# yanyan-li/Structure-SLAM-PointLine

Measured on AMD Instinct MI355X. Metric: front-end frames/sec (ORB+LSD extract+match) 640x480 @1000kp/200ln, higher is better.
Workload: dtype u8; 1 GPU; BASELINE configs[2]: 640x480 ORB(1000kp,8 levels)+LSD/LBD(<=200 lines) extract + Hamming match vs previous frame, inputs resident in HBM; batch_per_gpu=12288, global_batch=12288, unique_frames=64, streams=point branch and line branch on two HIP streams, parallelism=single GPU

## Files before the change

structure-slam-pointline_amd/csrc/lbd.h:

```cpp
#pragma once

template <class KeyPtr>
__device__ __forceinline__ void keyline_sort(KeyPtr keys, int P2, int tid) {
    for (int k = 2; k <= P2; k <<= 1)
        for (int j = k >> 1; j > 0; j >>= 1) {
            for (int i = tid; i < P2; i += 256) {
                int ixj = i ^ j;
                if (ixj > i) {
                    unsigned long long a = keys[i], c = keys[ixj];
                    bool up = (i & k) == 0;
                    if ((a > c) == up) { keys[i] = c; keys[ixj] = a; }
                }
            }
            __syncthreads();
        }
}

constexpr int KL_LDS = 1024;
__global__ __launch_bounds__(256) void k_keylines(uint8_t* __restrict__ ws, LsdPlan P, int maxLines,
                                                  sslam_keyline* __restrict__ klOut, double* __restrict__ fnOut,
                                                  int* __restrict__ counts, int cap) {
    __shared__ unsigned long long keysL[KL_LDS];
    const int b = blockIdx.x, tid = threadIdx.x;
    uint8_t* base = ws + (size_t)b * P.frameBytes;
// ... 33 lines not shown
        const float W = (float)P.w, H = (float)P.h;
        if (e0 < 0) e0 = 0; if (e0 >= W) e0 = W - 1.0f;
        if (e2 < 0) e2 = 0; if (e2 >= W) e2 = W - 1.0f;
        if (e1 < 0) e1 = 0; if (e1 >= H) e1 = H - 1.0f;
        if (e3 < 0) e3 = 0; if (e3 >= H) e3 = H - 1.0f;
        sslam_keyline k;
        k.startPointX = e0; k.startPointY = e1; k.endPointX = e2; k.endPointY = e3;
        k.sPointInOctaveX = e0; k.sPointInOctaveY = e1; k.ePointInOctaveX = e2; k.ePointInOctaveY = e3;
        const double ddx = (double)__fsub_rn(e0, e2), ddy = (double)__fsub_rn(e1, e3);
        k.lineLength = (float)sqrt(ddx * ddx + ddy * ddy);
        const int ax = cv_roundf(e0), ay = cv_roundf(e1), bx = cv_roundf(e2), by = cv_roundf(e3);
        k.numOfPixels = max(abs(bx - ax), abs(by - ay)) + 1;
        k.angle = (float)atan2((double)__fsub_rn(e3, e1), (double)__fsub_rn(e2, e0));
        k.class_id = i; k.octave = 0;
        k.size = __fmul_rn(__fsub_rn(e2, e0), __fsub_rn(e3, e1));
        k.response = __fdiv_rn(k.lineLength, (float)max(P.w, P.h));
        k.pt_x = __fdiv_rn(__fadd_rn(e2, e0), 2.f); k.pt_y = __fdiv_rn(__fadd_rn(e3, e1), 2.f);
        klw[i] = k;
        const unsigned long long key = ((unsigned long long)(~__float_as_uint(k.response)) << 32) | (unsigned)i;
        if (inLds) keysL[i] = key; else keysG[i] = key;
    }
    __syncthreads();
    int nOut = n;
    const bool doSort = n > maxLines;
    if (doSort) {
        int P2 = 1; while (P2 < n) P2 <<= 1;
        if (inLds) {
            for (int i = n + tid; i < P2; i += 256) keysL[i] = ~0ull;
            __syncthreads();
            keyline_sort(keysL, P2, tid);
        } else {
            for (int i = n + tid; i < P2; i += 256) keysG[i] = ~0ull;
            __syncthreads();
            keyline_sort(keysG, P2, tid);
        }
        nOut = maxLines;
    }
    nOut = min(nOut, cap);
    for (int i = tid; i < nOut; i += 256) {
        const int src = doSort ? (int)(unsigned)(inLds ? keysL[i] : keysG[i]) : i;
        sslam_keyline k = klw[src];
        if (doSort) k.class_id = i;
        klOut[(size_t)b * cap + i] = k;
        ((float2*)(base + P.offLbdDir))[i] = make_float2((float)cos((double)k.angle), (float)sin((double)k.angle));
        const double sx = k.startPointX, sy = k.startPointY, ex = k.endPointX, ey = k.endPointY;
        const double l0 = __dsub_rn(sy, ey), l1 = __dsub_rn(ex, sx), l2 = __dsub_rn(__dmul_rn(sx, ey), __dmul_rn(sy, ex));
        const double nrm = sqrt(__dadd_rn(__dmul_rn(l0, l0), __dmul_rn(l1, l1)));
        double* f = fnOut + ((size_t)b * cap + i) * 3;
        f[0] = l0 / nrm; f[1] = l1 / nrm; f[2] = l2 / nrm;
    }
    if (tid == 0) { counts[b] = nOut; misc->nKl = nOut; }
}

__global__ __launch_bounds__(256) void k_blur_sobel(const uint8_t* __restrict__ src, size_t spitch, size_t sframe, int w, int h,
                                                    unsigned* __restrict__ dxyo, size_t dframeBytes,
                                                    const int* __restrict__ tapsArr) {
    constexpr int R = 3;
    const int ngroups = (w + 3) >> 2;
    const int t = blockIdx.x * 256 + threadIdx.x;
    const int strip = t / ngroups, x4 = (t - strip * ngroups) * 4, y0 = strip * STRIP;
    if (y0 >= h) return;
    const int b = blockIdx.y;
    const uint8_t* s = src + (size_t)b * sframe;
    unsigned taps[5];
#pragma unroll
    for (int k = 0; k < 5; ++k) taps[k] = (unsigned)tapsArr[k];
    const unsigned T0 = taps[0] | (taps[1] << 8) | (taps[2] << 16) | (taps[3] << 24), T1 = taps[4];
    const bool fast = x4 >= 4 && x4 + 8 <= w && ((spitch | (size_t)(uintptr_t)s) & 3) == 0;
    const bool vec = ((w & 3) == 0) && ((dframeBytes & 15) == 0);
    unsigned hb[5][6];
    int bl[3][6];
    constexpr int NR = STRIP + 2 * R;
    const bool uni = row12_uniform(s, spitch, w);
    const int x4u = uni ? x4 : 0;
    Row12 ring[ROW_AHEAD_SOBEL];
#pragma unroll
    for (int k = 0; k < ROW_AHEAD_SOBEL; ++k) ring[k] = row12_issue(s, spitch, reflect_row(y0 - R + k, h, R), x4u, w);
#pragma unroll
    for (int r = 0; r < NR; ++r) {
        if (r >= 2 * R && y0 + r - 2 * R >= h) break;
        Row12 cur = ring[r % ROW_AHEAD_SOBEL];
        if (r + ROW_AHEAD_SOBEL < NR) ring[r % ROW_AHEAD_SOBEL] = row12_issue(s, spitch, reflect_row(y0 - R + r + ROW_AHEAD_SOBEL, h, R), x4u, w);
        row12_fix(cur, x4u, w);
        if (!uni) load_row12(s, spitch, reflect_row(y0 - R + r, h, R), x4, w, fast, cur.d0, cur.d1, cur.d2);
        const unsigned d0 = cur.d0, d1 = cur.d1, d2 = cur.d2;
#pragma unroll
        for (int c = 0; c < 6; ++c) hb[r % 5][c] = hdot(d0, d1, d2, c + 1, T0, T1);
        if (r >= 4) {
            const int q = r - 4;
#pragma unroll
            for (int c = 0; c < 6; ++c) {
                unsigned acc = 0;
#pragma unroll
                for (int k = 0; k < 5; ++k) acc = __umul24(hb[(q + k) % 5][c], taps[k]) + acc;
                bl[q % 3][c] = (int)min((acc + 32768u) >> 16, 255u);
            }
            if (q >= 2) {
                const int y = y0 + q - 2;
                const int* A = bl[(q - 2) % 3];
                const int* M = bl[(q - 1) % 3];
                const int* C = bl[q % 3];
                short gx[4], gy[4];
#pragma unroll
                for (int j = 0; j < 4; ++j) {
                    gx[j] = (short)((A[j + 2] - A[j]) + 2 * (M[j + 2] - M[j]) + (C[j + 2] - C[j]));
                    gy[j] = (short)((C[j] - A[j]) + 2 * (C[j + 1] - A[j + 1]) + (C[j + 2] - A[j + 2]));
                }
                unsigned* op = (unsigned*)((uint8_t*)dxyo + (size_t)b * dframeBytes) + (size_t)y * w + x4;
                unsigned pk[4];
#pragma unroll
                for (int j = 0; j < 4; ++j) pk[j] = ((unsigned)(unsigned short)gx[j]) | ((unsigned)(unsigned short)gy[j] << 16);
                if (x4 + 3 < w && vec) *(uint4*)op = make_uint4(pk[0], pk[1], pk[2], pk[3]);
                else {
#pragma unroll
                    for (int j = 0; j < 4; ++j) if (x4 + j < w) op[j] = pk[j];
                }
            }
        }
    }
}

__constant__ float kGaussL[21];
__constant__ float kGaussL2[21];
__constant__ float kGaussG[63];
__constant__ signed char kComb[64];

typedef float f32x2 __attribute__((ext_vector_type(2)));
__device__ __forceinline__ int cvt_rpi(float x) { int r; asm("v_cvt_rpi_i32_f32 %0, %1" : "=v"(r) : "v"(x)); return r; }
__device__ __forceinline__ f32x2 pk_mul_lo(f32x2 a, f32x2 b) { f32x2 r; asm("v_pk_mul_f32 %0, %1, %2 op_sel:[0,0] op_sel_hi:[1,0]" : "=v"(r) : "v"(a), "v"(b)); return r; }
__device__ __forceinline__ f32x2 pk_mul_hi_swapped(f32x2 a, f32x2 b) { f32x2 r; asm("v_pk_mul_f32 %0, %1, %2 op_sel:[1,1] op_sel_hi:[0,1]" : "=v"(r) : "v"(a), "v"(b)); return r; }
__device__ __forceinline__ f32x2 pk_add_sub(f32x2 a, f32x2 b) { f32x2 r; asm("v_pk_add_f32 %0, %1, %2 neg_hi:[0,1]" : "=v"(r) : "v"(a), "v"(b)); return r; }
__device__ __forceinline__ f32x2 pk_sub(f32x2 a, f32x2 b) { f32x2 r; asm("v_pk_add_f32 %0, %1, %2 neg_lo:[0,1] neg_hi:[0,1]" : "=v"(r) : "v"(a), "v"(b)); return r; }
__device__ __forceinline__ float max0(float x) { float r; asm("v_max_f32 %0, 0, %1" : "=v"(r) : "v"(x)); return r; }
__device__ __forceinline__ int med3_0(int x, int hi) { int r; asm("v_med3_i32 %0, %1, 0, %2" : "=v"(r) : "v"(x), "s"(hi)); return r; }
__device__ __forceinline__ f32x2 pk_mul(f32x2 a, f32x2 b) { f32x2 r; asm("v_pk_mul_f32 %0, %1, %2" : "=v"(r) : "v"(a), "v"(b)); return r; }
__device__ __forceinline__ f32x2 pk_add(f32x2 a, f32x2 b) { f32x2 r; asm("v_pk_add_f32 %0, %1, %2" : "=v"(r) : "v"(a), "v"(b)); return r; }

#ifdef SSLAM_TESTING
__global__ __launch_bounds__(256) void k_selftest_lbd_round(unsigned long long* __restrict__ bad) {
    unsigned long long nb0 = 0, nb1 = 0;
    const unsigned base = (blockIdx.x * 256u + threadIdx.x) << 8;
    for (unsigned i = 0; i < 256u; ++i) {
        const float x = __uint_as_float(base + i);
        if (!(fabsf(x) < 24608.f)) continue;
        const int t = (int)__fadd_rn(x, x);
        const int o = (int)(short)((t + 1) >> 1), n = cvt_rpi(x);
        const int Ws[3] = {0, 639, 16383};
#pragma unroll
        for (int k = 0; k < 3; ++k) nb0 += (min(max(o, 0), Ws[k]) != min(max(n, 0), Ws[k])) ? 1 : 0;
        if (x >= 0.f) nb1 += (n != (int)roundf(x)) ? 1 : 0;
    }
    if (nb0) atomicAdd(bad, nb0);
    if (nb1) atomicAdd(bad + 1, nb1);
}
#endif
constexpr int LBD_TB = 8;
template <bool RPI>
__global__ __launch_bounds__(64) void k_lbd(const uint8_t* __restrict__ ws, LsdPlan P, const sslam_keyline* __restrict__ kls,
                                            const int* __restrict__ counts, uint8_t* __restrict__ descOut, int cap) {
    constexpr int TB = LBD_TB, TN = TB, TP = TB + 1;
    __shared__ unsigned tbuf[64 * TP];
    float (*rows)[64] = (float (*)[64])&tbuf[0];
    static_assert(8 * 64 <= 64 * TP, "rows[][] lies over the walk's block array");
    __shared__ float band[8][NUM_BANDS];
    __shared__ float des[72];
    const int li = blockIdx.x, b = blockIdx.y, lane = threadIdx.x;
    if (li >= counts[b]) return;
    const uint8_t* base = ws + (size_t)b * P.frameBytes;
    const unsigned* dxyImg = (const unsigned*)(base + P.offDxy);
    const sslam_keyline kl = kls[(size_t)b * cap + li];
    const int lengthOfLSP = (short)kl.numOfPixels;
// ... 177 lines not shown
```

structure-slam-pointline_amd/csrc/lines.hip:

```cpp
#include "common.h"
#include <cmath>
#include <cstdlib>
#include <cfloat>
#include <algorithm>

namespace sslam { int launch_nfa_stream(sslam_ctx* ctx, hipStream_t st, uint8_t* ws, const void* plan, size_t planBytes, const double* lgam, uint8_t* clArea, size_t clFrameBytes,
                                        size_t stageOff, int nframes, int waves, long long spinTicks, bool besideCore); }
namespace sslam { int launch_nfa_stage(sslam_ctx* ctx, hipStream_t st, uint8_t* ws, const void* plan, size_t planBytes, const double* lgam, int nframes); }

using namespace sslam;

namespace {

#include "lsd_plan.h"
#include "lsd_front.h"
#include "lsd_regions.h"
#include "lsd_cluster.h"
#include "lsd_nfa.h"
#include "lbd.h"

__global__ void k_zero_misc(uint8_t* ws, LsdPlan P) {
    Misc* m = (Misc*)(ws + (size_t)blockIdx.x * P.frameBytes + P.offMisc);
    if (threadIdx.x == 0) {
        m->maxS = 0; m->nDefined = 0; m->nSeg = 0; m->nCand = 0; m->nKl = 0; m->overflow = 0; m->claim = 0;
// ... 119 lines not shown
    };
    P.nfaVariant = L->nfaVariant; P.lbdBitOrder = L->lbdBitOrder; P.lsdResize = L->lsdResize;
    P.tabX = 0; if (P.lsdResize) coeffs_linear(w, P.sw); else coeffs(SCALE, w, P.sw);
    P.tabY = (int)tabs.size(); if (P.lsdResize) coeffs_linear(h, P.sh); else coeffs(SCALE, h, P.sh);
    int rc;
    if ((rc = L->dTabs.ensure(tabs.size() * sizeof(int)))) return rc;
    SSLAM_HIP(hipMemcpy(L->dTabs.p, tabs.data(), tabs.size() * sizeof(int), hipMemcpyHostToDevice));
    int taps[16] = {0};
    for (int i = 0; i < 7; ++i) taps[i] = t7[i];
    for (int i = 0; i < 5; ++i) taps[8 + i] = t5[i];
    if ((rc = L->dTaps.ensure(sizeof(taps)))) return rc;
    SSLAM_HIP(hipMemcpy(L->dTaps.p, taps, sizeof(taps), hipMemcpyHostToDevice));
    size_t off = 0;
    auto take = [&](size_t bytes) { size_t o = off; off = align_up(off + bytes, 256); return o; };
    const size_t bpitch = ((size_t)w + 63) & ~(size_t)63;
    P.offBlur = take(bpitch * h);
    P.tW = P.sw; P.cW = P.sw;
    P.offT = take(sizeof(float) * (size_t)P.npx);
    P.offS = take(sizeof(int) * (size_t)P.npx);
    P.offCs = take(sizeof(float2) * (size_t)P.npx);
    P.offOrder = take(sizeof(unsigned) * (size_t)P.npx);
    P.offTileHist = take(sizeof(int) * (size_t)P.nTiles * N_BINS);
    P.offReg = take(sizeof(unsigned) * std::max((size_t)P.npx, (size_t)P.sh * P.nXB * 256));
    P.offComp = P.offReg;
    P.offSegCnt = take(sizeof(int) * (size_t)P.sh * P.nXB);
    P.offSorted = take(sizeof(unsigned) * (size_t)P.sh * P.nXB * 256);
    P.offSeg = take(sizeof(float4) * MAX_SEG);
    P.offCand = take(sizeof(double) * 12 * MAX_SEG);
    P.offFlag = take(sizeof(int) * MAX_SEG);
    P.offNfa = take(sizeof(NfaState) * MAX_SEG);
    P.offMisc = take(sizeof(Misc));
    P.offDxy = take(sizeof(unsigned) * (size_t)w * h);
    P.offKl = take(sizeof(sslam_keyline) * MAX_SEG);
    P.offLbdDir = take(sizeof(float2) * MAX_SEG);
    P.frameBytes = align_up(off, 4096);
    if (!L->dGtab.p) {
        if ((rc = L->dGtab.ensure(sizeof(float4) * ((size_t)GT * GT + 1)))) return rc;
        int* dSmin = (int*)(L->dGtab.as<float4>() + (size_t)GT * GT);
        const int big = 0x7FFFFFFF;
        SSLAM_HIP(hipMemcpy(dSmin, &big, sizeof(int), hipMemcpyHostToDevice));
        hipLaunchKernelGGL(k_grad_table, dim3((GT * GT + 255) / 256), dim3(256), 0, L->ctx->stream, L->dGtab.as<float4>(), P.rho);
        hipLaunchKernelGGL(k_grad_smin, dim3((2 * 510 * 510 + 256) / 256), dim3(256), 0, L->ctx->stream, dSmin, P.rho);
        SSLAM_HIP(hipStreamSynchronize(L->ctx->stream));
        SSLAM_HIP(hipMemcpy(&L->sMin, dSmin, sizeof(int), hipMemcpyDeviceToHost));
    }
    P.sMin = L->sMin;
    {
        const int nl = P.npx + 4;
        if ((rc = L->dLgam.ensure(sizeof(double) * (2 * (size_t)nl + 48)))) return rc;
        if ((rc = upload_nfa_tables(L->dLgam.as<double>(), nl, L->ctx->stream))) return rc;
    }
    {
        bool ok = (w % 4) == 0 && (P.sw % 4) == 0 && (P.sh % 4) == 0 && w == 5 * (P.sw / 4) && h == 5 * (P.sh / 4) && w >= 20 && h >= 10 && t7[0] == 0 && t7[6] == 0;
        for (int x = 0; ok && x < P.sw; ++x) ok = tabs[(size_t)P.tabX + 2 * x] == 5 * (x >> 2) + (x & 3);
        for (int y = 0; ok && y < P.sh; ++y) ok = tabs[(size_t)P.tabY + 2 * y] == 5 * (y >> 2) + (y & 3);
        L->fusedGeometry = ok;
    }
    L->planW = w; L->planH = h; L->wsFrames = 0;
    return SSLAM_OK;
}

extern "C" int sslam_lines_create(sslam_ctx* ctx, int max_lines, sslam_lines** out) {
    if (!ctx || !out || max_lines <= 0 || max_lines > MAX_SEG) { set_error("sslam_lines_create: invalid arguments"); return SSLAM_ERR_INVALID; }
    sslam_lines* L = new sslam_lines();
    L->ctx = ctx; L->maxLines = max_lines;
    *out = L;
    return SSLAM_OK;
}

extern "C" int sslam_lines_set_blur_variant(sslam_lines* L, int variant) {
    if (!L || (variant != 0 && variant != 1)) { set_error("sslam_lines_set_blur_variant: invalid arguments"); return SSLAM_ERR_INVALID; }
    std::lock_guard<std::recursive_mutex> lk(L->ctx->mu);
    if (L->blurVariant != variant) { L->blurVariant = variant; L->planW = L->planH = 0; }
    return SSLAM_OK;
}

static int lines_set_variant(sslam_lines* L, int which, int variant, const char* name) {
    if (!L || (variant != 0 && variant != 1)) { set_error("%s: invalid arguments", name); return SSLAM_ERR_INVALID; }
    std::lock_guard<std::recursive_mutex> lk(L->ctx->mu);
    int& field = which == 0 ? L->nfaVariant : which == 1 ? L->lbdBitOrder : which == 2 ? L->lsdResize : L->seedOrder;
    if (field != variant) { field = variant; L->planW = L->planH = 0; }
    return SSLAM_OK;
}
extern "C" int sslam_lines_set_nfa_variant(sslam_lines* L, int variant) { return lines_set_variant(L, 0, variant, "sslam_lines_set_nfa_variant"); }
extern "C" int sslam_lines_set_lbd_bit_order(sslam_lines* L, int variant) { return lines_set_variant(L, 1, variant, "sslam_lines_set_lbd_bit_order"); }
extern "C" int sslam_lines_set_resize_variant(sslam_lines* L, int variant) { return lines_set_variant(L, 2, variant, "sslam_lines_set_resize_variant"); }
extern "C" int sslam_lines_set_seed_order(sslam_lines* L, int variant) { return lines_set_variant(L, 3, variant, "sslam_lines_set_seed_order"); }

static int lines_host_seed_order(sslam_lines* L, uint8_t* ws, int nframes, hipStream_t st) {
    const LsdPlan& P = L->plan;
    struct NormPoint { int x, y, norm; };
    std::vector<int> S((size_t)P.npx);
    std::vector<NormPoint> pts;
    std::vector<unsigned> order;
    SSLAM_HIP(hipStreamSynchronize(st));
    for (int b = 0; b < nframes; ++b) {
        uint8_t* base = ws + (size_t)b * P.frameBytes;
        Misc m;
        SSLAM_HIP(hipMemcpy(&m, base + P.offMisc, sizeof(m), hipMemcpyDeviceToHost));
        SSLAM_HIP(hipMemcpy(S.data(), base + P.offS, sizeof(int) * (size_t)P.npx, hipMemcpyDeviceToHost));
        const double maxGrad = m.maxS > 0 ? std::sqrt((double)m.maxS / 4.0) : -1.0;
        const double binCoef = maxGrad > 0 ? (double)(N_BINS - 1) / maxGrad : 0.0;
        pts.clear(); pts.reserve((size_t)(P.sw - 1) * (P.sh - 1));
        for (int y = 0; y < P.sh - 1; ++y)
            for (int x = 0; x < P.sw - 1; ++x) pts.push_back({x, y, (int)(std::sqrt((double)S[(size_t)y * P.sw + x] / 4.0) * binCoef)});
        std::sort(pts.begin(), pts.end(), [](const NormPoint& a, const NormPoint& c) { return a.norm > c.norm; });
        order.clear();
// ... 42 lines not shown
enum class CoreForm {
    ClusterStream,
    Cluster,
    Lone,
    Guest,
    PerFrame,
    SixWave,
};

constexpr int CL_MAXFRAMES = 64;

static CoreForm lines_core_form(const sslam_lines* L, const LsdPlan& P, int nframes, const LinesKnobs& K, int* grid) {
    if (K.cluster && nframes <= CL_MAXFRAMES && P.sw <= TorusGlobal::XMASK + 1 && P.sh <= TorusGlobal::YMASK + 1)
        return K.nfaStreamWaves ? CoreForm::ClusterStream : CoreForm::Cluster;
    if (K.lone >= 0 ? K.lone != 0 : nframes < 1024) return CoreForm::Lone;
    if (lines_guest_form(L, nframes, K, grid)) return CoreForm::Guest;
    return nframes <= 16 * L->ctx->num_cus ? CoreForm::PerFrame : CoreForm::SixWave;
}

extern "C" int sslam_lines_destroy(sslam_lines* L) {
    if (!L) return SSLAM_OK;
    (void)hipSetDevice(L->ctx->device);
    (void)hipStreamSynchronize(L->ctx->stream);
    if (L->nfaStream) { (void)hipStreamSynchronize(L->nfaStream); (void)hipStreamDestroy(L->nfaStream); (void)hipEventDestroy(L->nfaFork); (void)hipEventDestroy(L->nfaJoin); }
    DevBuf* bufs[] = {&L->dWs, &L->dCl, &L->dTabs, &L->dTaps, &L->dLgam, &L->dGtab, &L->dImg, &L->dKl, &L->dDesc, &L->dFn, &L->dCounts};
    for (DevBuf* b : bufs) b->release();
    L->hOut.release();
    delete L;
    return SSLAM_OK;
}

struct LinesCall {
    sslam_lines* L; const LsdPlan& P; const uint8_t* images; size_t pitch, imageStride; int nframes; hipStream_t st; uint8_t* ws;
};

struct SideJoin {
    sslam_lines* L; hipStream_t st; bool forked = false, joined = false;
    void join() { if (forked && !joined) { (void)hipEventRecord(L->nfaJoin, L->nfaStream); (void)hipStreamWaitEvent(st, L->nfaJoin, 0); joined = true; } }
    ~SideJoin() { join(); }
};

static int lines_side_stream_ready(sslam_lines* L) {
    if (!L->nfaStream) {
        SSLAM_HIP(hipStreamCreateWithFlags(&L->nfaStream, hipStreamNonBlocking));
        SSLAM_HIP(hipEventCreateWithFlags(&L->nfaFork, hipEventDisableTiming));
        SSLAM_HIP(hipEventCreateWithFlags(&L->nfaJoin, hipEventDisableTiming));
    }
    return SSLAM_OK;
}

static void lines_blur_sobel(const LinesCall& c, hipStream_t s) {
    const LsdPlan& P = c.P;
    sslam::ProfScope _ps(c.L->ctx, "k_blur_sobel", s);
    hipLaunchKernelGGL(k_blur_sobel, dim3((((P.w + 3) / 4) * ((P.h + STRIP - 1) / STRIP) + 255) / 256, c.nframes), dim3(256), 0, s, c.images, c.pitch, c.imageStride, P.w, P.h,
                       (unsigned*)(c.ws + P.offDxy), P.frameBytes, c.L->dTaps.as<int>() + 8);
}

static int lines_prologue(const LinesCall& c) {
    sslam_lines* L = c.L; const LsdPlan& P = c.P; hipStream_t st = c.st;
    const int* taps = L->dTaps.as<int>();
    const int* tabX = L->dTabs.as<int>() + P.tabX; const int* tabY = L->dTabs.as<int>() + P.tabY;
    const int mode = (P.lsdResize ? 1 : 0) | (L->seedOrder ? 2 : 0);
    const bool fused = L->fusedGeometry && GRAD_ROWS == 8 && ((uintptr_t)c.images & 3) == 0 && (c.pitch & 3) == 0 && (c.imageStride & 3) == 0 && c.pitch <= 0x7FFFFFFF;
    if (fused) {
        static decltype(&k_lsd_grad_fused<0>) const kGradFused[4] = {k_lsd_grad_fused<0>, k_lsd_grad_fused<1>, k_lsd_grad_fused<2>, k_lsd_grad_fused<3>};
        sslam::ProfScope _ps(L->ctx, "k_lsd_grad", st);
        const dim3 gg(P.nXB, (P.sh + 31) / 32, c.nframes);
        hipLaunchKernelGGL(kGradFused[mode], gg, dim3(64, 4), 0, st, c.images, c.pitch, c.imageStride, c.ws, P, L->dGtab.as<float4>(), tabX, tabY, taps, c.nframes);
    } else {
        static decltype(&k_lsd_grad<0>) const kGrad[4] = {k_lsd_grad<0>, k_lsd_grad<1>, k_lsd_grad<2>, k_lsd_grad<3>};
        const size_t bpitch = ((size_t)P.w + 63) & ~(size_t)63;
        { sslam::ProfScope _ps(L->ctx, "k_blur7", st); hipLaunchKernelGGL(k_blur7, dim3((((P.w + 3) / 4) * ((P.h + STRIP - 1) / STRIP) + 255) / 256, c.nframes), dim3(256), 0, st, c.images, c.pitch, c.imageStride,
                           c.ws + P.offBlur, bpitch, P.frameBytes, P.w, P.h, taps); }
        { sslam::ProfScope _ps(L->ctx, "k_lsd_grad", st);
          const dim3 gg(P.nXB, (P.sh + 4 * GRAD_ROWS - 1) / (4 * GRAD_ROWS), c.nframes);
          hipLaunchKernelGGL(kGrad[mode], gg, dim3(64, 4), 0, st, c.ws, P, L->dGtab.as<float4>(), bpitch, tabX, tabY); }
    }
    if (L->seedOrder) return lines_host_seed_order(L, c.ws, c.nframes, st);
    const bool runs = P.sw <= (1 << SORT_XY_BITS) && P.sh <= (1 << SORT_XY_BITS);
    const dim3 sg(sort_grid(P.nTiles, c.nframes));
    { sslam::ProfScope _ps(L->ctx, "k_lsd_hist", st); hipLaunchKernelGGL(runs ? k_lsd_hist_sort : k_lsd_hist, sg, dim3(64), 0, st, c.ws, P, c.nframes); }
    { sslam::ProfScope _ps(L->ctx, "k_lsd_scan", st); hipLaunchKernelGGL(k_lsd_scan, dim3(c.nframes), dim3(1024), 0, st, c.ws, P); }
    { sslam::ProfScope _ps(L->ctx, "k_lsd_scatter", st); hipLaunchKernelGGL(runs ? k_lsd_scatter_runs : k_lsd_scatter, sg, dim3(64), 0, st, c.ws, P, c.nframes); }
    return SSLAM_OK;
}

static int lines_core_cluster(const LinesCall& c, const LinesKnobs& K, bool streamNfa, SideJoin& side, size_t* nfaStageOff) {
    sslam_lines* L = c.L; const LsdPlan& P = c.P; const int nframes = c.nframes; hipStream_t st = c.st;
    int rc;
    const bool bigFrame = P.sw > TorusFrame::XMASK + 1 || P.sh > TorusFrame::YMASK + 1;
    const int window = K.clWindow, clShift = K.clSmap;
    int nWG = K.clWgs;
    const int clSpecWords = clShift < 0 ? 0 : (((P.sw + (1 << clShift) - 1) >> clShift) * ((P.sh + (1 << clShift) - 1) >> clShift) + 31) / 32;
    const size_t maxSubs = ((size_t)P.npx + CL_SUB - 1) / CL_SUB;
    const size_t zeroBytes = 512 + ((maxSubs * sizeof(ClSub) + 511) & ~(size_t)511) + 4 * (size_t)((clSpecWords + 127) & ~127) + (bigFrame ? 4 * (size_t)TorusGlobal::WORDS : 0);
    if (nframes > 8) nWG = std::max(2, std::min(nWG, 32 / ((nframes + 7) / 8)));
    const size_t stageOff = zeroBytes + maxSubs * CL_RES * sizeof(ClRec) + 4 * (size_t)CL_ARENA * (size_t)std::max(1, (nWG - 1) * CL_HPW);
    const size_t clFrame = align_up(stageOff + (streamNfa ? sizeof(double) * 12 * (size_t)MAX_SEG : 0), 4096);
    L->clFrame = clFrame; L->clSlots = nframes;
    const size_t clSlots = (size_t)nframes;
    if (L->dCl.cap < clFrame * clSlots) { SSLAM_HIP(hipStreamSynchronize(st)); if ((rc = L->dCl.ensure(clFrame * clSlots))) return rc; }
    for (int f = 0; f < nframes; ++f) SSLAM_HIP(hipMemsetAsync(L->dCl.as<uint8_t>() + (size_t)f * clFrame, 0, zeroBytes, st));
    const size_t clLds = sizeof(unsigned) * std::max((size_t)QCAP + 4 + (bigFrame ? 0 : TorusFrame::WORDS) + CL_SCAN + CL_RING_WORDS, (size_t)CL_HPW * (CL_LIST + ClTorus::WORDS));
    const auto kern = streamNfa ? k_lsd_regions_cl<1> : k_lsd_regions_cl<0>;
    const dim3 grd(8 * nWG * ((nframes + 7) / 8));
    SSLAM_HIP(hipFuncSetAttribute((const void*)kern, hipFuncAttributeMaxDynamicSharedMemorySize, (int)clLds));
    if (!streamNfa) {
        hipLaunchKernelGGL(kern, grd, dim3(64 * CL_WAVES), clLds, st, c.ws, P, L->dCl.as<uint8_t>(), clFrame, nframes, nWG, clSpecWords, clShift, window);
// ... 460 lines not shown
```

structure-slam-pointline_amd/csrc/lsd_front.h:

```cpp
#pragma once

constexpr int STRIP = 32;

__device__ __forceinline__ void load_row12(const uint8_t* __restrict__ s, size_t spitch, int yy, int x4, int w, bool fast, unsigned& d0, unsigned& d1, unsigned& d2) {
    const uint8_t* row = s + (size_t)yy * spitch;
    if (fast) {
        const unsigned* q = (const unsigned*)(row + x4 - 4);
        d0 = q[0]; d1 = q[1]; d2 = q[2];
    } else {
        unsigned px[12];
#pragma unroll
        for (int i = 0; i < 12; ++i) {
            int xx = reflect101(min(x4 - 4 + i, w + 2), w);
            xx = min(max(xx, 0), w - 1);
            px[i] = row[xx];
        }
        d0 = px[0] | (px[1] << 8) | (px[2] << 16) | (px[3] << 24);
        d1 = px[4] | (px[5] << 8) | (px[6] << 16) | (px[7] << 24);
        d2 = px[8] | (px[9] << 8) | (px[10] << 16) | (px[11] << 24);
    }
}
struct Row12 { unsigned d0, d1, d2; };
constexpr int ROW_AHEAD_BLUR7 = 1, ROW_AHEAD_SOBEL = 2;
__device__ __forceinline__ bool row12_uniform(const uint8_t* s, size_t spitch, int w) { return (w & 3) == 0 && w >= 12 && ((spitch | (size_t)(uintptr_t)s) & 3) == 0; }
// ... 183 lines not shown
                float4* c = (float4*)(Cs + i);
                c[0] = make_float4(cs[0].x, cs[0].y, cs[1].x, cs[1].y);
                c[1] = make_float4(cs[2].x, cs[2].y, cs[3].x, cs[3].y);
            }
        } else {
#pragma unroll
            for (int j = 0; j < 4; ++j) if (x4 + j < P.sw) {
                T[i + j] = ang[j];
                if (DENSE) S[i + j] = sv[j];
                if (flags & (1u << j)) { S[i + j] = sv[j]; Cs[i + j] = cs[j]; }
            }
        }
        const int seg = y * P.nXB + blockIdx.x;
        const int cnt = __popc(flags), incl = wave_incl_scan(cnt);
        unsigned* dst = comp + ((size_t)seg << 8);
        int pos = incl - cnt;
#pragma unroll
        for (int j = 0; j < 4; ++j) if (flags & (1u << j)) dst[pos++] = ((unsigned)sv[j] << 8) | (unsigned)(4 * lane + j);
        if (lane == 63) segCnt[seg] = incl;
#pragma unroll
        for (int j = 0; j < 4; ++j) if (!DENSE || (flags & (1u << j))) smax = max(smax, sv[j]);
    };
    int pc[5], pn[5];
    if (fast) {
        unsigned d0[2][3], d1[2][3];
        load_raw(yBeg, d0); load_raw(min(yBeg + 1, P.sh - 1), d1);
        scale_fast(yBeg, d0, pc);
        for (int y = yBeg; y < yEnd; ++y) {
            scale_fast(min(y + 1, P.sh - 1), d1, pn);
            load_raw(min(y + 2, P.sh - 1), d1);
            process(y, pc, pn);
#pragma unroll
            for (int j = 0; j < 5; ++j) pc[j] = pn[j];
        }
    } else {
        scale_slow(yBeg, pc);
        for (int y = yBeg; y < yEnd; ++y) {
            scale_slow(min(y + 1, P.sh - 1), pn);
            process(y, pc, pn);
#pragma unroll
            for (int j = 0; j < 5; ++j) pc[j] = pn[j];
        }
    }
    smax = wave_max(smax);
    if (lane == 0 && smax > 0) atomicMax(&misc->maxS, smax);
}


struct Raw16 { unsigned v[4]; };
template <int MODE>
__global__ __launch_bounds__(256) void k_lsd_grad_fused(const uint8_t* __restrict__ img, size_t ipitch, size_t iframe, const uint8_t* __restrict__ ws, LsdPlan P,
                                                        const float4* __restrict__ gtab, const int* __restrict__ tx, const int* __restrict__ ty, const int* __restrict__ tapsArr, int nframes) {
    constexpr bool LIN = (MODE & 1) != 0, DENSE = (MODE & 2) != 0;
    for (int b = blockIdx.z; b < nframes; b += gridDim.z) {
    const uint8_t* base = ws + (size_t)b * P.frameBytes;
    const uint8_t* src = img + (size_t)b * iframe;
    float* T = (float*)(base + P.offT);
    float2* Cs = (float2*)(base + P.offCs);
    int* S = (int*)(base + P.offS); (void)S;
    Misc* misc = (Misc*)(base + P.offMisc);
    unsigned* comp = (unsigned*)(base + P.offComp);
    int* segCnt = (int*)(base + P.offSegCnt);
    const int lane = threadIdx.x;
    const int strip = __builtin_amdgcn_readfirstlane(blockIdx.y * 4 + threadIdx.y);
    const int yBeg = strip * 8, yEnd = min(P.sh, yBeg + 8);
    if (yBeg >= P.sh) return;
    const int x4 = (blockIdx.x * 64 + lane) * 4;
    const bool inx = x4 < P.sw;
    const int x4c = min(x4, P.sw - 4);
    const int c0 = (x4c >> 2) * 5;
    unsigned cx[5];
#pragma unroll
    for (int j = 0; j < 5; ++j) cx[j] = (unsigned)((const int2*)tx)[min(x4c + j, P.sw - 1)].y;
    const int2* tyv = (const int2*)ty;
    const int a = (c0 - 2) & ~3;
    const unsigned o0 = (unsigned)(c0 - 2) & 3u;
    const bool isLeft = a < 0, isRight = a + 8 >= P.w;
    const int aLoad = isLeft ? 0 : a;
    const unsigned t1 = (unsigned)tapsArr[1], t2 = (unsigned)tapsArr[2], t3 = (unsigned)tapsArr[3], t4 = (unsigned)tapsArr[4], t5 = (unsigned)tapsArr[5];
    const unsigned TA = t1 | (t2 << 8) | (t3 << 16) | (t4 << 24);
    unsigned Hring[5][4];
    const int off2 = min(aLoad + 8, P.w - 4), off3 = min(aLoad + 12, P.w - 4);
    auto raw_row = [&](int n) -> Raw16 {
        const int rr = reflect_row(10 * strip - 2 + n, P.h, 2);
        const uint8_t* row = src + (size_t)rr * ipitch;
        Raw16 r;
        const uint2 lo = *(const uint2*)(row + aLoad);
        r.v[0] = lo.x; r.v[1] = lo.y; r.v[2] = *(const unsigned*)(row + off2); r.v[3] = *(const unsigned*)(row + off3);
        return r;
    };
    auto hrow = [&](const Raw16& r, unsigned (&Hp)[4]) {
        unsigned L0 = r.v[0], L1 = r.v[1], L2 = r.v[2], L3 = r.v[3];
        if (isLeft) {
            L3 = L2; L2 = L1; L1 = L0;
            L0 = __builtin_amdgcn_perm(L2, L1, 0x01020304u);
        }
        if (isRight) L2 = __builtin_amdgcn_perm(L1, L0, 0x03040506u);
        const unsigned e0 = __builtin_amdgcn_alignbyte(L1, L0, o0), e1 = __builtin_amdgcn_alignbyte(L2, L1, o0), e2 = __builtin_amdgcn_alignbyte(L3, L2, o0);
        unsigned H[8];
#pragma unroll
        for (int i = 0; i < 7; ++i) {
            const int q = i >> 2, sft = i & 3;
            const unsigned lo = q == 0 ? (sft ? __builtin_amdgcn_alignbyte(e1, e0, (unsigned)sft) : e0) : (sft ? __builtin_amdgcn_alignbyte(e2, e1, (unsigned)sft) : e1);
            const int i4 = i + 4, q4 = i4 >> 2, s4 = i4 & 3;
            const unsigned b4 = ((q4 == 1 ? e1 : e2) >> (8 * s4)) & 255u;
            H[i] = __builtin_amdgcn_udot4(lo, TA, __umul24(b4, t5), false);
        }
        H[7] = 0;
#pragma unroll
        for (int j = 0; j < 4; ++j) Hp[j] = H[2 * j] | (H[2 * j + 1] << 16);
    };
    auto blur_row = [&](int top, int (&B)[7]) {
#pragma unroll
        for (int i = 0; i < 7; ++i) {
            unsigned acc = 32768u;
#pragma unroll
            for (int k = 0; k < 5; ++k) {
                const unsigned hp = Hring[(top + k) % 5][i >> 1];
                const unsigned tk = k == 0 ? t1 : k == 1 ? t2 : k == 2 ? t3 : k == 3 ? t4 : t5;
                acc += __umul24((i & 1) ? (hp >> 16) : (hp & 0xFFFFu), tk);
            }
            B[i] = (int)min(acc >> 16, 255u);
        }
    };
    auto scale_row = [&](int yy, const int (&B0)[7], const int (&B1)[7], int (&p)[5]) {
        const unsigned cy = (unsigned)tyv[yy].y;
#pragma unroll
        for (int j = 0; j < 5; ++j) {
            const int i = j < 4 ? j : 5;
            p[j] = scaled_px<LIN>((unsigned)B0[i] | ((unsigned)B0[i + 1] << 8), (unsigned)B1[i] | ((unsigned)B1[i + 1] << 8), cx[j], cy);
        }
        if (x4c + 4 > P.sw - 1) p[4] = p[3];
    };
    int smax = 0;
    auto process = [&](int y, const int (&p0)[5], const int (&p1)[5]) {
        float ang[4]; float2 cs[4]; int sv[4], gidx[4];
        unsigned flags = 0;
        const bool lastRow = y >= P.sh - 1;
#pragma unroll
        for (int j = 0; j < 4; ++j) {
            ang[j] = NOTDEF_F; cs[j] = make_float2(0.f, 0.f); sv[j] = -1;
            const int DA = p1[j + 1] - p0[j], BC = p0[j + 1] - p1[j];
            const int gx = DA + BC, gy = DA - BC, s = gx * gx + gy * gy;
            gidx[j] = (gy + 510) * GT + (gx + 510);
            if (inx && !lastRow && x4 + j < P.sw - 1 && s >= P.sMin) { flags |= 1u << j; sv[j] = s; }
            else if (DENSE) sv[j] = s;
        }
#pragma unroll
        for (int j = 0; j < 4; ++j)
            if (flags & (1u << j)) { const float4 rec = gtab[gidx[j]]; ang[j] = rec.x; cs[j] = make_float2(rec.y, rec.z); }
        const size_t i = (size_t)y * P.sw + x4;
        if (inx) *(float4*)(T + i) = make_float4(ang[0], ang[1], ang[2], ang[3]);
        if (DENSE && inx) *(int4*)(S + i) = make_int4(sv[0], sv[1], sv[2], sv[3]);
        if (flags) {
            if (!DENSE) *(int4*)(S + i) = make_int4(sv[0], sv[1], sv[2], sv[3]);
            float4* c = (float4*)(Cs + i);
            c[0] = make_float4(cs[0].x, cs[0].y, cs[1].x, cs[1].y);
            c[1] = make_float4(cs[2].x, cs[2].y, cs[3].x, cs[3].y);
        }
        const int seg = y * P.nXB + blockIdx.x;
        const int cnt = __popc(flags), incl = wave_incl_scan(cnt);
        unsigned* dst = comp + ((size_t)seg << 8);
        int pos = incl - cnt;
#pragma unroll
        for (int j = 0; j < 4; ++j) if (flags & (1u << j)) dst[pos++] = ((unsigned)sv[j] << 8) | (unsigned)(4 * lane + j);
        if (lane == 63) segCnt[seg] = incl;
#pragma unroll
        for (int j = 0; j < 4; ++j) if (!DENSE || (flags & (1u << j))) smax = max(smax, sv[j]);
    };
    int Bprev[7], Bcur[7], pc[5], pn[5];
    constexpr int AH = 2;
    Raw16 ring[AH];
#pragma unroll
    for (int k = 0; k < AH; ++k) ring[k] = raw_row(k);
#pragma unroll
    for (int n = 0; n < 16; ++n) {
        const Raw16 cur = ring[n % AH];
        if (n + AH < 16) ring[n % AH] = raw_row(n + AH);
        hrow(cur, Hring[n % 5]);
        if (n < 4) continue;
        const int bi = n - 4;
        blur_row((n + 1) % 5, Bcur);
        const int sIdx = bi == 1 ? 0 : bi == 2 ? 1 : bi == 3 ? 2 : bi == 4 ? 3 : bi == 6 ? 4 : bi == 7 ? 5 : bi == 8 ? 6 : bi == 9 ? 7 : bi == 11 ? 8 : -1;
        if (sIdx >= 0) {
            const int yy = min(yBeg + sIdx, P.sh - 1);
            if (sIdx == 0) scale_row(yy, Bprev, Bcur, pc);
            else {
                if (yBeg + sIdx > P.sh - 1) {
#pragma unroll
                    for (int j = 0; j < 5; ++j) pn[j] = pc[j];
                } else scale_row(yy, Bprev, Bcur, pn);
                const int y = yBeg + sIdx - 1;
                if (y < yEnd) process(y, pc, pn);
#pragma unroll
                for (int j = 0; j < 5; ++j) pc[j] = pn[j];
            }
        }
#pragma unroll
        for (int i = 0; i < 7; ++i) Bprev[i] = Bcur[i];
    }
    smax = wave_max(smax);
    if (lane == 0 && smax > 0) atomicMax(&misc->maxS, smax);
    }
}

__device__ __forceinline__ int lsd_bin(int s, double binCoef) {
    int i = (int)(sqrt((double)s / 4.0) * binCoef);
    return min(max(i, 0), N_BINS - 1);
}
__device__ __forceinline__ double lsd_bin_coef(int maxS) {
    return maxS > 0 ? (double)(N_BINS - 1) / sqrt((double)maxS / 4.0) : 0.0;
}
__device__ __forceinline__ int lsd_bin_wave(int s, bool have, double binCoef, float coef32) {
    const float y = __builtin_amdgcn_sqrtf((float)s) * coef32;
    const float fl = floorf(y), fr = y - fl;
    int i = (int)fl;
    const bool amb = have && !(fr >= 1e-3f && fr <= 0.999f && y < (float)(N_BINS - 2));
    if (__builtin_amdgcn_ballot_w64(amb)) { if (amb) i = lsd_bin(s, binCoef); }
    return i;
}

#ifdef SSLAM_TESTING
__global__ __launch_bounds__(256) void k_selftest_lsd_bin(int maxS, unsigned long long* __restrict__ bad) {
    const double bc = lsd_bin_coef(maxS); const float bc32 = (float)(bc * 0.5);
    unsigned long long nb = 0;
    for (long long s0 = (long long)blockIdx.x * 256; s0 <= maxS; s0 += (long long)gridDim.x * 256) {
        const long long s = s0 + threadIdx.x;
        const bool have = s <= maxS;
        const int a = lsd_bin_wave(have ? (int)s : 0, have, bc, bc32);
        if (have && a != lsd_bin((int)s, bc)) ++nb;
    }
    if (nb) atomicAdd(bad, nb);
}
#endif

constexpr int MAX_TSEG = 256;
__device__ __forceinline__ int tile_segments(const int* __restrict__ segCnt, int seg0, int nseg, int* __restrict__ pref, int lane) {
    int carry = 0;
    for (int s0 = 0; s0 < nseg; s0 += 64) {
        const int s = s0 + lane;
        const int c = s < nseg ? segCnt[seg0 + s] : 0;
        const int incl = wave_incl_scan(c);
        if (s < nseg) pref[s] = carry + incl - c;
        carry += __builtin_amdgcn_readlane(incl, 63);
    }
    if (lane == 0) pref[nseg] = carry;
    return carry;
}

__device__ __forceinline__ bool sort_tile(int nTiles, int nframes, int& tile, int& b) {
    const int xcd = blockIdx.x & 7, k = blockIdx.x >> 3, q = k / nTiles;
    tile = k - q * nTiles; b = q * 8 + xcd;
// ... 242 lines not shown
```

Measured before the change: 82220 frames/s.

## Persist blur-sobel across frames and stage LSD gradient stores through LDS

k_blur_sobel becomes a persistent kernel that loops over frames, with a grid sized from the CU count. Its row loop becomes a rolled outer loop over an unrolled six-row body, which keeps the ring indices static and cuts code size. In the fused LSD gradient kernel, the compacted candidate list and the cos/sin pairs are staged in LDS per wave, then written out as coalesced row stores instead of scattered per-lane stores. Blurred rows are packed into bytes to save registers, and the x-coefficient table is assumed periodic, guarded by an extra host-side geometry check. These trade extra LDS traffic and wave barriers for fewer kernel blocks and better global write coalescing.

```diff
diff --git a/structure-slam-pointline_amd/csrc/lbd.h b/structure-slam-pointline_amd/csrc/lbd.h
--- a/structure-slam-pointline_amd/csrc/lbd.h
+++ b/structure-slam-pointline_amd/csrc/lbd.h
@@ -109,71 +109,79 @@
     if (tid == 0) { counts[b] = nOut; misc->nKl = nOut; }
 }
 
+constexpr int SOBEL_BODY = 6;
 __global__ __launch_bounds__(256) void k_blur_sobel(const uint8_t* __restrict__ src, size_t spitch, size_t sframe, int w, int h,
                                                     unsigned* __restrict__ dxyo, size_t dframeBytes,
-                                                    const int* __restrict__ tapsArr) {
+                                                    const int* __restrict__ tapsArr, int nframes) {
     constexpr int R = 3;
+    constexpr int NR = STRIP + 2 * R, U = SOBEL_BODY;
+    static_assert(U >= 6 && U % 3 == 0 && U % ROW_AHEAD_SOBEL == 0, "the body keeps the indices of all three rings static");
     const int ngroups = (w + 3) >> 2;
     const int t = blockIdx.x * 256 + threadIdx.x;
     const int strip = t / ngroups, x4 = (t - strip * ngroups) * 4, y0 = strip * STRIP;
     if (y0 >= h) return;
-    const int b = blockIdx.y;
-    const uint8_t* s = src + (size_t)b * sframe;
     unsigned taps[5];
 #pragma unroll
     for (int k = 0; k < 5; ++k) taps[k] = (unsigned)tapsArr[k];
     const unsigned T0 = taps[0] | (taps[1] << 8) | (taps[2] << 16) | (taps[3] << 24), T1 = taps[4];
+    const bool vec = ((w & 3) == 0) && ((dframeBytes & 15) == 0);
+    const int rEnd = min(NR, h - y0 + 2 * R);
+    for (int b = blockIdx.y; b < nframes; b += gridDim.y) {
+    const uint8_t* s = src + (size_t)b * sframe;
     const bool fast = x4 >= 4 && x4 + 8 <= w && ((spitch | (size_t)(uintptr_t)s) & 3) == 0;
-    const bool vec = ((w & 3) == 0) && ((dframeBytes & 15) == 0);
-    unsigned hb[5][6];
+    unsigned hb[U][6];
     int bl[3][6];
-    constexpr int NR = STRIP + 2 * R;
     const bool uni = row12_uniform(s, spitch, w);
     const int x4u = uni ? x4 : 0;
+    unsigned* const oframe = (unsigned*)((uint8_t*)dxyo + (size_t)b * dframeBytes) + x4;
     Row12 ring[ROW_AHEAD_SOBEL];
 #pragma unroll
     for (int k = 0; k < ROW_AHEAD_SOBEL; ++k) ring[k] = row12_issue(s, spitch, reflect_row(y0 - R + k, h, R), x4u, w);
-#pragma unroll
-    for (int r = 0; r < NR; ++r) {
-        if (r >= 2 * R && y0 + r - 2 * R >= h) break;
-        Row12 cur = ring[r % ROW_AHEAD_SOBEL];
-        if (r + ROW_AHEAD_SOBEL < NR) ring[r % ROW_AHEAD_SOBEL] = row12_issue(s, spitch, reflect_row(y0 - R + r + ROW_AHEAD_SOBEL, h, R), x4u, w);
-        row12_fix(cur, x4u, w);
-        if (!uni) load_row12(s, spitch, reflect_row(y0 - R + r, h, R), x4, w, fast, cur.d0, cur.d1, cur.d2);
-        const unsigned d0 = cur.d0, d1 = cur.d1, d2 = cur.d2;
-#pragma unroll
-        for (int c = 0; c < 6; ++c) hb[r % 5][c] = hdot(d0, d1, d2, c + 1, T0, T1);
-        if (r >= 4) {
-            const int q = r - 4;
-#pragma unroll
-            for (int c = 0; c < 6; ++c) {
-                unsigned acc = 0;
-#pragma unroll
-                for (int k = 0; k < 5; ++k) acc = __umul24(hb[(q + k) % 5][c], taps[k]) + acc;
-                bl[q % 3][c] = (int)min((acc + 32768u) >> 16, 255u);
-            }
-            if (q >= 2) {
-                const int y = y0 + q - 2;
-                const int* A = bl[(q - 2) % 3];
-                const int* M = bl[(q - 1) % 3];
-                const int* C = bl[q % 3];
-                short gx[4], gy[4];
-#pragma unroll
-                for (int j = 0; j < 4; ++j) {
-                    gx[j] = (short)((A[j + 2] - A[j]) + 2 * (M[j + 2] - M[j]) + (C[j + 2] - C[j]));
-                    gy[j] = (short)((C[j] - A[j]) + 2 * (C[j + 1] - A[j + 1]) + (C[j + 2] - A[j + 2]));
+#pragma unroll 1
+    for (int rb = 0; rb < rEnd; rb += U) {
+#pragma unroll
+        for (int u = 0; u < U; ++u) {
+            const int r = rb + u;
+            if (r >= rEnd) break;
+            Row12 cur = ring[u % ROW_AHEAD_SOBEL];
+            if (r + ROW_AHEAD_SOBEL < rEnd) ring[u % ROW_AHEAD_SOBEL] = row12_issue(s, spitch, reflect_row(y0 - R + r + ROW_AHEAD_SOBEL, h, R), x4u, w);
+            row12_fix(cur, x4u, w);
+            if (!uni) load_row12(s, spitch, reflect_row(y0 - R + r, h, R), x4, w, fast, cur.d0, cur.d1, cur.d2);
+            const unsigned d0 = cur.d0, d1 = cur.d1, d2 = cur.d2;
+#pragma unroll
+            for (int c = 0; c < 6; ++c) hb[u][c] = hdot(d0, d1, d2, c + 1, T0, T1);
+            if (r >= 4) {
+#pragma unroll
+                for (int c = 0; c < 6; ++c) {
+                    unsigned acc = 0;
+#pragma unroll
+                    for (int k = 0; k < 5; ++k) acc = __umul24(hb[(u + 2 + k) % U][c], taps[k]) + acc;
+                    bl[(u + 2) % 3][c] = (int)min((acc + 32768u) >> 16, 255u);
                 }
-                unsigned* op = (unsigned*)((uint8_t*)dxyo + (size_t)b * dframeBytes) + (size_t)y * w + x4;
-                unsigned pk[4];
-#pragma unroll
-                for (int j = 0; j < 4; ++j) pk[j] = ((unsigned)(unsigned short)gx[j]) | ((unsigned)(unsigned short)gy[j] << 16);
-                if (x4 + 3 < w && vec) *(uint4*)op = make_uint4(pk[0], pk[1], pk[2], pk[3]);
-                else {
-#pragma unroll
-                    for (int j = 0; j < 4; ++j) if (x4 + j < w) op[j] = pk[j];
+                if (r >= 6) {
+                    const int y = y0 + r - 6;
+                    const int* A = bl[u % 3];
+                    const int* M = bl[(u + 1) % 3];
+                    const int* C = bl[(u + 2) % 3];
+                    short gx[4], gy[4];
+#pragma unroll
+                    for (int j = 0; j < 4; ++j) {
+                        gx[j] = (short)((A[j + 2] - A[j]) + 2 * (M[j + 2] - M[j]) + (C[j + 2] - C[j]));
+                        gy[j] = (short)((C[j] - A[j]) + 2 * (C[j + 1] - A[j + 1]) + (C[j + 2] - A[j + 2]));
+                    }
+                    unsigned* op = oframe + (size_t)y * w;
+                    unsigned pk[4];
+#pragma unroll
+                    for (int j = 0; j < 4; ++j) pk[j] = ((unsigned)(unsigned short)gx[j]) | ((unsigned)(unsigned short)gy[j] << 16);
+                    if (x4 + 3 < w && vec) *(uint4*)op = make_uint4(pk[0], pk[1], pk[2], pk[3]);
+                    else {
+#pragma unroll
+                        for (int j = 0; j < 4; ++j) if (x4 + j < w) op[j] = pk[j];
+                    }
                 }
             }
         }
+    }
     }
 }
 
diff --git a/structure-slam-pointline_amd/csrc/lines.hip b/structure-slam-pointline_amd/csrc/lines.hip
--- a/structure-slam-pointline_amd/csrc/lines.hip
+++ b/structure-slam-pointline_amd/csrc/lines.hip
@@ -195,7 +195,7 @@
     }
     {
         bool ok = (w % 4) == 0 && (P.sw % 4) == 0 && (P.sh % 4) == 0 && w == 5 * (P.sw / 4) && h == 5 * (P.sh / 4) && w >= 20 && h >= 10 && t7[0] == 0 && t7[6] == 0;
-        for (int x = 0; ok && x < P.sw; ++x) ok = tabs[(size_t)P.tabX + 2 * x] == 5 * (x >> 2) + (x & 3);
+        for (int x = 0; ok && x < P.sw; ++x) ok = tabs[(size_t)P.tabX + 2 * x] == 5 * (x >> 2) + (x & 3) && tabs[(size_t)P.tabX + 2 * x + 1] == tabs[(size_t)P.tabX + 2 * (x & 3) + 1];
         for (int y = 0; ok && y < P.sh; ++y) ok = tabs[(size_t)P.tabY + 2 * y] == 5 * (y >> 2) + (y & 3);
         L->fusedGeometry = ok;
     }
@@ -344,8 +344,10 @@
 static void lines_blur_sobel(const LinesCall& c, hipStream_t s) {
     const LsdPlan& P = c.P;
     sslam::ProfScope _ps(c.L->ctx, "k_blur_sobel", s);
-    hipLaunchKernelGGL(k_blur_sobel, dim3((((P.w + 3) / 4) * ((P.h + STRIP - 1) / STRIP) + 255) / 256, c.nframes), dim3(256), 0, s, c.images, c.pitch, c.imageStride, P.w, P.h,
-                       (unsigned*)(c.ws + P.offDxy), P.frameBytes, c.L->dTaps.as<int>() + 8);
+    const int gx = (((P.w + 3) / 4) * ((P.h + STRIP - 1) / STRIP) + 255) / 256;
+    const int gy = std::max(1, std::min(c.nframes, 32 * c.L->ctx->num_cus / gx));
+    hipLaunchKernelGGL(k_blur_sobel, dim3(gx, gy), dim3(256), 0, s, c.images, c.pitch, c.imageStride, P.w, P.h,
+                       (unsigned*)(c.ws + P.offDxy), P.frameBytes, c.L->dTaps.as<int>() + 8, c.nframes);
 }
 
 static int lines_prologue(const LinesCall& c) {
diff --git a/structure-slam-pointline_amd/csrc/lsd_front.h b/structure-slam-pointline_amd/csrc/lsd_front.h
--- a/structure-slam-pointline_amd/csrc/lsd_front.h
+++ b/structure-slam-pointline_amd/csrc/lsd_front.h
@@ -259,15 +259,12 @@
 __global__ __launch_bounds__(256) void k_lsd_grad_fused(const uint8_t* __restrict__ img, size_t ipitch, size_t iframe, const uint8_t* __restrict__ ws, LsdPlan P,
                                                         const float4* __restrict__ gtab, const int* __restrict__ tx, const int* __restrict__ ty, const int* __restrict__ tapsArr, int nframes) {
     constexpr bool LIN = (MODE & 1) != 0, DENSE = (MODE & 2) != 0;
+    __shared__ uint4 csStageAll[4][128];
+    __shared__ unsigned compStageAll[4][256];
+    uint4* const csStage = csStageAll[threadIdx.y];
+    unsigned* const compStage = compStageAll[threadIdx.y];
+    auto lds_order = []() { __builtin_amdgcn_fence(__ATOMIC_SEQ_CST, "wavefront"); __builtin_amdgcn_wave_barrier(); };
     for (int b = blockIdx.z; b < nframes; b += gridDim.z) {
-    const uint8_t* base = ws + (size_t)b * P.frameBytes;
-    const uint8_t* src = img + (size_t)b * iframe;
-    float* T = (float*)(base + P.offT);
-    float2* Cs = (float2*)(base + P.offCs);
-    int* S = (int*)(base + P.offS); (void)S;
-    Misc* misc = (Misc*)(base + P.offMisc);
-    unsigned* comp = (unsigned*)(base + P.offComp);
-    int* segCnt = (int*)(base + P.offSegCnt);
     const int lane = threadIdx.x;
     const int strip = __builtin_amdgcn_readfirstlane(blockIdx.y * 4 + threadIdx.y);
     const int yBeg = strip * 8, yEnd = min(P.sh, yBeg + 8);
@@ -278,7 +275,7 @@
     const int c0 = (x4c >> 2) * 5;
     unsigned cx[5];
 #pragma unroll
-    for (int j = 0; j < 5; ++j) cx[j] = (unsigned)((const int2*)tx)[min(x4c + j, P.sw - 1)].y;
+    for (int j = 0; j < 5; ++j) cx[j] = (unsigned)((const int2*)tx)[j].y;
     const int2* tyv = (const int2*)ty;
     const int a = (c0 - 2) & ~3;
     const unsigned o0 = (unsigned)(c0 - 2) & 3u;
@@ -288,6 +285,14 @@
     const unsigned TA = t1 | (t2 << 8) | (t3 << 16) | (t4 << 24);
     unsigned Hring[5][4];
     const int off2 = min(aLoad + 8, P.w - 4), off3 = min(aLoad + 12, P.w - 4);
+    const uint8_t* base = ws + (size_t)b * P.frameBytes;
+    const uint8_t* src = img + (size_t)b * iframe;
+    float* T = (float*)(base + P.offT);
+    float2* Cs = (float2*)(base + P.offCs);
+    int* S = (int*)(base + P.offS); (void)S;
+    Misc* misc = (Misc*)(base + P.offMisc);
+    unsigned* comp = (unsigned*)(base + P.offComp);
+    int* segCnt = (int*)(base + P.offSegCnt);
     auto raw_row = [&](int n) -> Raw16 {
         const int rr = reflect_row(10 * strip - 2 + n, P.h, 2);
         const uint8_t* row = src + (size_t)rr * ipitch;
@@ -317,7 +322,8 @@
 #pragma unroll
         for (int j = 0; j < 4; ++j) Hp[j] = H[2 * j] | (H[2 * j + 1] << 16);
     };
-    auto blur_row = [&](int top, int (&B)[7]) {
+    auto blur_row = [&](int top, unsigned (&Bp)[2]) {
+        unsigned B[7];
 #pragma unroll
         for (int i = 0; i < 7; ++i) {
             unsigned acc = 32768u;
@@ -327,15 +333,19 @@
                 const unsigned tk = k == 0 ? t1 : k == 1 ? t2 : k == 2 ? t3 : k == 3 ? t4 : t5;
                 acc += __umul24((i & 1) ? (hp >> 16) : (hp & 0xFFFFu), tk);
             }
-            B[i] = (int)min(acc >> 16, 255u);
-        }
-    };
-    auto scale_row = [&](int yy, const int (&B0)[7], const int (&B1)[7], int (&p)[5]) {
+            B[i] = min(acc >> 16, 255u);
+        }
+        Bp[0] = B[0] | (B[1] << 8) | (B[2] << 16) | (B[3] << 24); Bp[1] = B[4] | (B[5] << 8) | (B[6] << 16);
+    };
+    auto pair = [](const unsigned (&Bp)[2], int i) -> unsigned {
+        return i < 3 ? Bp[0] >> (8 * i) : i == 3 ? __builtin_amdgcn_alignbyte(Bp[1], Bp[0], 3u) : Bp[1] >> (8 * (i - 4));
+    };
+    auto scale_row = [&](int yy, const unsigned (&B0)[2], const unsigned (&B1)[2], int (&p)[5]) {
         const unsigned cy = (unsigned)tyv[yy].y;
 #pragma unroll
         for (int j = 0; j < 5; ++j) {
             const int i = j < 4 ? j : 5;
-            p[j] = scaled_px<LIN>((unsigned)B0[i] | ((unsigned)B0[i + 1] << 8), (unsigned)B1[i] | ((unsigned)B1[i + 1] << 8), cx[j], cy);
+            p[j] = scaled_px<LIN>(pair(B0, i), pair(B1, i), cx[j], cy);
         }
         if (x4c + 4 > P.sw - 1) p[4] = p[3];
     };
@@ -353,29 +363,48 @@
             if (inx && !lastRow && x4 + j < P.sw - 1 && s >= P.sMin) { flags |= 1u << j; sv[j] = s; }
             else if (DENSE) sv[j] = s;
         }
-#pragma unroll
-        for (int j = 0; j < 4; ++j)
-            if (flags & (1u << j)) { const float4 rec = gtab[gidx[j]]; ang[j] = rec.x; cs[j] = make_float2(rec.y, rec.z); }
         const size_t i = (size_t)y * P.sw + x4;
-        if (inx) *(float4*)(T + i) = make_float4(ang[0], ang[1], ang[2], ang[3]);
+        const int seg = y * P.nXB + blockIdx.x;
+        const int cnt = __popc(flags), incl = wave_incl_scan(cnt);
+        const unsigned long long fm = __builtin_amdgcn_ballot_w64(flags != 0);
+        lds_order();
         if (DENSE && inx) *(int4*)(S + i) = make_int4(sv[0], sv[1], sv[2], sv[3]);
         if (flags) {
             if (!DENSE) *(int4*)(S + i) = make_int4(sv[0], sv[1], sv[2], sv[3]);
-            float4* c = (float4*)(Cs + i);
-            c[0] = make_float4(cs[0].x, cs[0].y, cs[1].x, cs[1].y);
-            c[1] = make_float4(cs[2].x, cs[2].y, cs[3].x, cs[3].y);
-        }
-        const int seg = y * P.nXB + blockIdx.x;
-        const int cnt = __popc(flags), incl = wave_incl_scan(cnt);
-        unsigned* dst = comp + ((size_t)seg << 8);
-        int pos = incl - cnt;
-#pragma unroll
-        for (int j = 0; j < 4; ++j) if (flags & (1u << j)) dst[pos++] = ((unsigned)sv[j] << 8) | (unsigned)(4 * lane + j);
+            int pos = incl - cnt;
+#pragma unroll
+            for (int j = 0; j < 4; ++j) if (flags & (1u << j)) compStage[pos++] = ((unsigned)sv[j] << 8) | (unsigned)(4 * lane + j);
+        }
+#pragma unroll
+        for (int j = 0; j < 4; ++j) if (!DENSE || (flags & (1u << j))) smax = max(smax, sv[j]);
+        lds_order();
+        if (fm) {
+            const int total = __builtin_amdgcn_readlane(incl, 63);
+            unsigned* dst = comp + ((size_t)seg << 8);
+#pragma unroll
+            for (int k = 0; k < 4; ++k) {
+                if (64 * k >= total) break;
+                if (64 * k + lane < total) dst[64 * k + lane] = compStage[64 * k + lane];
+            }
+        }
         if (lane == 63) segCnt[seg] = incl;
 #pragma unroll
-        for (int j = 0; j < 4; ++j) if (!DENSE || (flags & (1u << j))) smax = max(smax, sv[j]);
-    };
-    int Bprev[7], Bcur[7], pc[5], pn[5];
+        for (int j = 0; j < 4; ++j)
+            if (flags & (1u << j)) { const float4 rec = gtab[gidx[j]]; ang[j] = rec.x; cs[j] = make_float2(rec.y, rec.z); }
+        if (inx) *(float4*)(T + i) = make_float4(ang[0], ang[1], ang[2], ang[3]);
+        if (flags) {
+            csStage[2 * lane] = make_uint4(__float_as_uint(cs[0].x), __float_as_uint(cs[0].y), __float_as_uint(cs[1].x), __float_as_uint(cs[1].y));
+            csStage[2 * lane + 1] = make_uint4(__float_as_uint(cs[2].x), __float_as_uint(cs[2].y), __float_as_uint(cs[3].x), __float_as_uint(cs[3].y));
+        }
+        lds_order();
+        if (fm) {
+            uint4* crow = (uint4*)(Cs + (size_t)y * P.sw + (size_t)blockIdx.x * 256);
+            if ((fm >> (lane >> 1)) & 1) crow[lane] = csStage[lane];
+            if ((fm >> (32 + (lane >> 1))) & 1) crow[64 + lane] = csStage[64 + lane];
+        }
+    };
+    unsigned Bprev[2], Bcur[2];
+    int pc[5], pn[5];
     constexpr int AH = 2;
     Raw16 ring[AH];
 #pragma unroll
@@ -403,8 +432,7 @@
                 for (int j = 0; j < 5; ++j) pc[j] = pn[j];
             }
         }
-#pragma unroll
-        for (int i = 0; i < 7; ++i) Bprev[i] = Bcur[i];
+        Bprev[0] = Bcur[0]; Bprev[1] = Bcur[1];
     }
     smax = wave_max(smax);
     if (lane == 0 && smax > 0) atomicMax(&misc->maxS, smax);
```

Result: no change. 82440 frames/s (median of 6 runs) (+0.3%).
